# SrikarK-code/clip-dplm

Measured on NVIDIA B200. Metric: contrastive_fwd_bwd_pairs_per_sec, higher is better.
Workload: dtype bf16

## Files before the change

### clip-dplm_b200/csrc/clipnce_api.cu

```cuda
#include <cuda.h>
#include <cuda_bf16.h>
#include <cuda_runtime.h>

#include <cmath>
#include <cstdarg>
#include <cstdio>
#include <cstdlib>
#include <cstring>
#include <mutex>
#include <set>
#include <string>
#include <utility>

#include "../../include/clipnce.h"
#include "kernels_aux.cuh"
#include "kernels_head.cuh"
#include "kernels_link.cuh"
#include "kernels_pair.cuh"
#include "kernels_pair2.cuh"
#include "kernels_simt.cuh"
#include "kernels_tc.cuh"

namespace {

// ... 1007 lines not shown
  if (world == 1 || world < 0 || world > pair2::MAX_WORLD) return false;
  if (world == 0 ? n_rows != n_cols : n_rows * world != n_cols) return false;
  const int64_t min_n = env_int("CLIPNCE_BWD2_MIN_N", 12288);
  if (n_rows % 128 != 0 || n_cols % 256 != 0 || n_rows * n_cols < min_n * min_n || n_cols > (1ll << 22)) return false;
  if (world >= 2 && (n_cols / world) % 256 != 0) return false;
  const int slots = pair_slots();
  if (slots < 8) return false;
  pl->n_rb = (int)(n_rows / 128);
  pl->n_steps = (int)(n_cols / 256);
  pl->n_half = (int)ceil_div(d, 256);
  const int forced_p = (int)env_int("CLIPNCE_BWD2_P", 0);
  const int forced_seg = (int)env_int("CLIPNCE_BWD2_SEG", 0);
  constexpr double r = 1.0;
  double best_t = 1e300;
  int best_p = 0, best_seg = 0;
  for (int n_seg = 1; n_seg <= 8; n_seg *= 2) {
    int ns = world >= 2 ? world : n_seg;
    if (world == 0 && forced_seg >= 1) ns = forced_seg;
    if (pl->n_steps % ns != 0) continue;
    const int seg_steps = pl->n_steps / ns;
    if (seg_steps < 8 && ns > 1 && world == 0 && forced_seg < 1) continue;
    const int64_t n_items = (int64_t)pl->n_rb * ns;
    const double slab_steps = (double)(ns - 1) * (double)n_rows * (double)d * 8.0 / 3e12 / 3.9e-6;
    const bool force = forced_p >= 1 && forced_p <= slots - 1;
    for (int Pe = force ? forced_p : slots / 2; Pe <= (force ? forced_p : slots - 2); ++Pe) {
      const int Q = slots - Pe;
      const double tp = (double)ceil_div(n_items, Pe) * ((double)seg_steps + 1.0);
      const double tc_ = (double)n_items * (double)seg_steps / ((double)Q * 2.0 * r);
      const double t = ((tp > tc_ ? tp : tc_) + slab_steps) * (world == 0 && ns > 1 ? 1.08 : 1.0);
      if (t < best_t - 1e-9) { best_t = t; best_p = Pe; best_seg = ns; }
    }
    if (world >= 2 || forced_seg >= 1) break;
  }
  if (best_p == 0) return false;
  pl->P = best_p;
  pl->Q = slots - best_p;
  pl->n_seg = best_seg;
  pl->seg_steps = pl->n_steps / best_seg;
  pl->n_items = pl->n_rb * best_seg;
  pl->n_rounds = (int)ceil_div(pl->n_items, pl->P);
  pl->depth = pair2::RING_DEPTH;
  const int nkc = (int)(d / 64);
  const int total = (pair::SMEM_LIMIT - pair2::producer_smem(nkc, 0)) / pair::STAGE_BYTES;
  if (total < 4) return false;
  auto cap = [](int v) { return v > pair2::MAXS ? pair2::MAXS : v; };
  pl->stages_b = cap(total / 2);
  pl->stages_a = cap(total - total / 2);
  pl->stages_c = cap((pair::SMEM_LIMIT - pair2::consumer_smem(0)) / pair2::C_STAGE);
  const int ps = pair2::producer_smem(nkc, pl->stages_a + pl->stages_b), cs = pair2::consumer_smem(pl->stages_c);
  pl->smem = ps > cs ? ps : cs;
  size_t off = 0;
  auto region = [&](size_t bytes) { const size_t o = off; off = (size_t)round_up((int64_t)(off + bytes), 256); return o; };
  pl->off_flags = region(sizeof(uint32_t) * 2 * (size_t)pl->n_rounds * (size_t)pl->seg_steps);
  pl->off_ring = region((size_t)pl->depth * (size_t)pl->P * 128 * 256 * 2);
  pl->off_dxh = region(sizeof(float) * (size_t)pl->n_seg * (size_t)n_rows * (size_t)d);
  pl->off_dyh = region(sizeof(float) * (size_t)n_cols * (size_t)d);
  pl->off_part = region(sizeof(float) * (size_t)ceil_div(n_rows > n_cols ? n_rows : n_cols, 8));
  pl->bytes = off;
  return true;
}

int bwd2_launch(const Bwd2Plan& pl, const void* x, const void* y, const float* rinv_x, const float* rinv_y, int64_t n_rows,
                int64_t n_cols, int64_t d, int64_t diag_offset, float scale, const float* scale_dev, const float* row_m,
                const float* row_w, const float* col_m, const float* col_w, float diag_w, char* ws, float* const* dy_peer,
                int world, cudaStream_t st) {
  uint32_t* flags_dev = reinterpret_cast<uint32_t*>(ws + pl.off_flags);
  const size_t n_flags = (size_t)pl.n_rounds * (size_t)pl.seg_steps;
  CUDA_TRY(cudaMemsetAsync(flags_dev, 0, sizeof(uint32_t) * 2 * n_flags, st));
  pair2::Params p;
  memset(&p, 0, sizeof p);
  p.n_rows = (int)n_rows; p.n_cols = (int)n_cols; p.d = (int)d;
  p.nkc = (int)(d / 64); p.nq2 = (int)ceil_div(d, 256); p.n_half = pl.n_half;
  p.nsbuf = p.nq2 <= 2 ? 2 : 1;
  p.n_rb = pl.n_rb; p.n_seg = pl.n_seg; p.seg_steps = pl.seg_steps; p.n_items = pl.n_items; p.n_rounds = pl.n_rounds;
  p.P = pl.P; p.Q = pl.Q; p.depth = pl.depth;
  p.stages_a = pl.stages_a; p.stages_b = pl.stages_b; p.stages_c = pl.stages_c;
  p.diag_offset = diag_offset; p.scale = scale; p.scale_dev = scale_dev; p.diag_w = diag_w;
  p.rinv_x = rinv_x; p.rinv_y = rinv_y; p.row_m = row_m; p.row_w = row_w; p.col_m = col_m; p.col_w = col_w;
  p.dx = reinterpret_cast<float*>(ws + pl.off_dxh);
  p.dy = reinterpret_cast<float*>(ws + pl.off_dyh);
  p.world = world;
  for (int s = 0; s < world; ++s) p.dy_peer[s] = dy_peer[s];
  p.ready = flags_dev; p.done = flags_dev + n_flags;
  CUtensorMap tx, ty, tyg, tg;
  int rc;
  if ((rc = make_tmap(&tx, x, d, n_rows, d, pair2::ROWS))) return rc;
  if ((rc = make_tmap(&ty, y, d, n_cols, d, 128))) return rc;
  if ((rc = make_tmap(&tyg, y, d, n_cols, d, 64))) return rc;
  if ((rc = make_tmap(&tg, ws + pl.off_ring, 256, (int64_t)pl.depth * pl.P * 128, 256, 64))) return rc;
  auto kern = tc_family(CLIPNCE_BF16, d, scale, 0) == 2 ? pair2::bwd2_kernel<true> : pair2::bwd2_kernel<false>;
  if ((rc = allow_smem(kern, pair::SMEM_LIMIT))) return rc;
  kern<<<2 * (pl.P + pl.Q), pair2::THREADS, pl.smem, st>>>(tx, ty, tyg, tg, p);
  CUDA_TRY(cudaGetLastError());
  return 0;
}
}

extern "C" {

int clipnce_backward_both_workspace_bytes(int64_t n_rows, int64_t n_cols, int64_t d, int dtype, float scale, int flags,
                                          int world, size_t* out) {
  if (!out) return fail(CLIPNCE_EINVAL, "backward_both_workspace_bytes: null pointer");
  Bwd2Plan pl;
  *out = (n_rows >= 1 && n_cols >= 1 && d >= 1 && bwd2_plan(n_rows, n_cols, d, dtype, scale, flags, world, &pl) &&
          check_device_sm100() == 0 && bwd2_device_ok()) ? pl.bytes : 0;
  return 0;
}

int clipnce_backward_both_dx(const void* x, const void* y, const float* rinv_x, const float* rinv_y, int64_t n,
                             int64_t d, float scale, const float* scale_dev, const float* row_m, const float* row_w,
                             const float* col_m, const float* col_w, float diag_w, int dtype, int flags,
                             const void* x_orig, const void* y_orig, int in_dtype, const float* grad_scale, void* dx,
                             void* dy, int out_dtype, float* d_scale_sum, void* workspace, size_t workspace_bytes,
                             void* stream) {
  if (!x || !y || !rinv_x || !rinv_y || !row_m || !row_w || !col_m || !col_w || !x_orig || !y_orig || !dx || !dy || !workspace)
    return fail(CLIPNCE_EINVAL, "backward_both_dx: null pointer");
  if ((in_dtype != CLIPNCE_BF16 && in_dtype != CLIPNCE_F32) || (out_dtype != CLIPNCE_BF16 && out_dtype != CLIPNCE_F32))
    return fail(CLIPNCE_EINVAL, "backward_both_dx: bad dtype");
  if (in_dtype == dtype && (x_orig != x || y_orig != y))
    return fail(CLIPNCE_EINVAL, "backward_both_dx: x_orig / y_orig of the compute type must be x / y themselves");
  if (!aligned16(x) || !aligned16(y) || !aligned16(workspace)) return fail(CLIPNCE_EINVAL, "backward_both_dx: operands must be 16-byte aligned");
  int rc = check_device_sm100();
  if (rc) return rc;
  Bwd2Plan pl;
  if (!bwd2_plan(n, n, d, dtype, scale, flags, 0, &pl) || !bwd2_device_ok())
    return fail(CLIPNCE_EUNSUPPORTED, "backward_both_dx: shape not served (see clipnce_backward_both_workspace_bytes)");
  if (workspace_bytes < pl.bytes) return fail(CLIPNCE_EWORKSPACE, "backward_both_dx: workspace %zu < %zu", workspace_bytes, pl.bytes);
  cudaStream_t st = as_stream(stream);
  char* ws = reinterpret_cast<char*>(workspace);
  if ((rc = bwd2_launch(pl, x, y, rinv_x, rinv_y, n, n, d, 0, scale, scale_dev, row_m, row_w, col_m, col_w, diag_w, ws, nullptr,
                        0, st)))
    return rc;
  float* ds_part = reinterpret_cast<float*>(ws + pl.off_part);
  const aux::FinishSide sx = finish_side(reinterpret_cast<float*>(ws + pl.off_dxh), pl.n_seg, n, d, x, x_orig, rinv_x, dx,
                                         d_scale_sum ? ds_part : nullptr);
  const aux::FinishSide sy = finish_side(reinterpret_cast<float*>(ws + pl.off_dyh), 1, n, d, y, y_orig, rinv_y, dy, nullptr);
  if ((rc = launch_finish(&sx, 1, n, d, CLIPNCE_BF16, in_dtype, out_dtype, grad_scale, true, st))) return rc;
  if ((rc = launch_finish(&sy, 1, n, d, CLIPNCE_BF16, in_dtype, out_dtype, grad_scale, true, st))) return rc;
  if (d_scale_sum) {
    aux::reduce_scalar_partials_par<<<1, 256, 0, st>>>(ds_part, (int)ceil_div(n, 8), 1.f, d_scale_sum);
    CUDA_TRY(cudaGetLastError());
  }
  return 0;
}

int clipnce_backward_both_sharded(const void* x, const void* y, const float* rinv_x, const float* rinv_y, int64_t n_rows,
                                  int64_t n_cols, int64_t d, int64_t diag_offset, float scale, const float* scale_dev,
                                  const float* row_m, const float* row_w, const float* col_m, const float* col_w,
                                  float diag_w, int dtype, int flags, void* const* peer_base, int world, int rank,
                                  int64_t slots_offset, void* workspace, size_t workspace_bytes, void* stream) {
  if (!x || !y || !rinv_x || !rinv_y || !row_m || !row_w || !col_m || !col_w || !workspace || !peer_base)
    return fail(CLIPNCE_EINVAL, "backward_both_sharded: null pointer");
  if (!aligned16(x) || !aligned16(y) || !aligned16(workspace)) return fail(CLIPNCE_EINVAL, "backward_both_sharded: operands must be 16-byte aligned");
  if (world < 2 || world > pair2::MAX_WORLD || rank < 0 || rank >= world || slots_offset < 0 || slots_offset % 16 != 0)
    return fail(CLIPNCE_EINVAL, "backward_both_sharded: bad world / rank / slots_offset");
  if (diag_offset != (int64_t)rank * n_rows) return fail(CLIPNCE_EINVAL, "backward_both_sharded: diag_offset must be rank * n_rows");
  int rc = check_device_sm100();
  if (rc) return rc;
  Bwd2Plan pl;
  if (!bwd2_plan(n_rows, n_cols, d, dtype, scale, flags, world, &pl) || !bwd2_device_ok())
    return fail(CLIPNCE_EUNSUPPORTED, "backward_both_sharded: shape not served (see clipnce_backward_both_workspace_bytes)");
  if (workspace_bytes < pl.bytes) return fail(CLIPNCE_EWORKSPACE, "backward_both_sharded: workspace %zu < %zu", workspace_bytes, pl.bytes);
  char* ws = reinterpret_cast<char*>(workspace);
  float* dy_peer[pair2::MAX_WORLD];
  for (int s = 0; s < world; ++s) {
    if (!peer_base[s] || !aligned16(peer_base[s])) return fail(CLIPNCE_EINVAL, "backward_both_sharded: peer buffer %d is null or unaligned", s);
// ... 346 lines not shown
```

### clip-dplm_b200/csrc/kernels_pair2.cuh

```cuda
#pragma once
#include "kernels_pair.cuh"

namespace pair2 {

using pair::LOG2E;
using pair::STAGE_BYTES;
using pair::STEP_J;
using pair::TMEM_COLS;

constexpr int THREADS = 416;
constexpr int STORE_WARP = 12;
constexpr int EPI_WARPS = 8;
constexpr int ROWS = 64;
constexpr int X_CHUNK = ROWS * 128;
constexpr int G_BYTES = 4 * 8192;
constexpr int SMALL = 10240;
constexpr int C_STAGE = 32768;
constexpr int MAXS = 6;
constexpr int RING_DEPTH = 16;
constexpr int MAX_WORLD = 16;

constexpr int B_FULL_A = 0, B_EMPTY_A = MAXS, B_FULL_B = 2 * MAXS, B_EMPTY_B = 3 * MAXS, B_XFULL = 4 * MAXS,
              B_XEMPTY = B_XFULL + 1, B_SFULL = B_XEMPTY + 1, B_SEMPTY = B_SFULL + 2, B_GFULL = B_SEMPTY + 2,
              B_GEMPTY = B_GFULL + 4, B_ACCFULL = B_GEMPTY + 4, B_ACCEMPTY = B_ACCFULL + 2, B_GSFULL = B_ACCEMPTY + 2,
              B_GSTORED = B_GSFULL + 4, B_COUNT = B_GSTORED + 4;
static_assert(B_COUNT * 8 <= 1000, "barrier block");

struct Params {
  int n_rows, n_cols, d;
  int nsbuf;
  int nkc, nq2, n_half;
  int n_rb, n_seg, seg_steps, n_items, n_rounds;
  int P, Q, depth;
  int stages_a, stages_b, stages_c;
  long long diag_offset;
  float scale, diag_w;
  const float* scale_dev;
  const float* rinv_x;
  const float* rinv_y;
  const float* row_m;
  const float* row_w;
  const float* col_m;
  const float* col_w;
  float* dx;
  float* dy;
  float* dy_peer[MAX_WORLD];
  int world;
  uint32_t* ready;
  uint32_t* done;
};

__host__ __device__ constexpr int producer_smem(int nkc, int stages) {
  return nkc * X_CHUNK + G_BYTES + stages * STAGE_BYTES + SMALL;
}
constexpr int FLUSH_BYTES = EPI_WARPS * 4096;
__host__ __device__ constexpr int consumer_smem(int stages) { return stages * C_STAGE + FLUSH_BYTES + SMALL; }
__device__ __forceinline__ float4 ld_shared_v4(uint32_t addr) {
  float4 v;
  asm volatile("ld.shared.v4.f32 {%0, %1, %2, %3}, [%4];" : "=f"(v.x), "=f"(v.y), "=f"(v.z), "=f"(v.w) : "r"(addr) : "memory");
  return v;
}

__device__ __forceinline__ void publish(uint32_t* flag) {
  ptx::fence_proxy_async_all();
  ptx::red_release_gpu_add(flag, 1u);
}

struct Sub {
  int seg, p_lo, p_hi, rb_lo;
  bool first, last;
};
__device__ __forceinline__ int round_items(const Params& p, int r) { return min(p.P, p.n_items - r * p.P); }
__device__ __forceinline__ int round_subs(const Params& p, int r) {
  const int lo = r * p.P, hi = lo + round_items(p, r);
  return (hi - 1) / p.n_rb - lo / p.n_rb + 1;
}
__device__ __forceinline__ Sub round_sub(const Params& p, int r, int k) {
  const int lo = r * p.P, hi = lo + round_items(p, r);
  Sub s;
  s.seg = lo / p.n_rb + k;
  const int a = max(lo, s.seg * p.n_rb), b = min(hi, (s.seg + 1) * p.n_rb);
  s.p_lo = a - lo;
  s.p_hi = b - lo;
  s.rb_lo = a - s.seg * p.n_rb;
  s.first = a == s.seg * p.n_rb;
  s.last = b == (s.seg + 1) * p.n_rb;
  return s;
}

template <bool TWO_EXP>
__global__ void __cluster_dims__(2, 1, 1) __launch_bounds__(THREADS, 1)
bwd2_kernel(const __grid_constant__ CUtensorMap tmap_x,
            const __grid_constant__ CUtensorMap tmap_y,
            const __grid_constant__ CUtensorMap tmap_yg,
            const __grid_constant__ CUtensorMap tmap_g,
            const Params p) {
  extern __shared__ __align__(1024) uint8_t smem[];
  const uint32_t base = ptx::smem_u32(smem);
  if ((base & 1023u) != 0) __trap();
  const uint32_t rank = ptx::cluster_ctarank();
  const bool leader = rank == 0;
  const int warp = threadIdx.x >> 5;
  const int lane = threadIdx.x & 31;
  const int pair_id = blockIdx.x >> 1;
  const bool is_producer = pair_id < p.P;

  const int body = max(producer_smem(p.nkc, p.stages_a + p.stages_b), consumer_smem(p.stages_c)) - SMALL;
  const uint32_t bars = base + body;
  auto bar = [&](int i) -> uint32_t { return bars + 8u * i; };
  volatile uint32_t* tmem_ptr_smem = reinterpret_cast<volatile uint32_t*>(smem + body + 1016);
  float* const colv = reinterpret_cast<float*>(smem + body + 1024);

  const float sc = p.scale_dev != nullptr ? __ldg(p.scale_dev) : p.scale;
  const float k2 = sc * LOG2E;

  if (warp == 0 && lane == 0) {
    ptx::prefetch_tmap(&tmap_x);
    ptx::prefetch_tmap(&tmap_y);
    ptx::prefetch_tmap(&tmap_yg);
    ptx::prefetch_tmap(&tmap_g);
  }
  if (warp == 1 && lane == 0) {
    for (int s = 0; s < MAXS; ++s) {
      ptx::mbar_init(bar(B_FULL_A + s), 1);
      ptx::mbar_init(bar(B_EMPTY_A + s), 1);
      ptx::mbar_init(bar(B_FULL_B + s), 1);
      ptx::mbar_init(bar(B_EMPTY_B + s), 1);
    }
    ptx::mbar_init(bar(B_XFULL), 1);
    ptx::mbar_init(bar(B_XEMPTY), 1);
    for (int b = 0; b < 2; ++b) {
      ptx::mbar_init(bar(B_SFULL + b), 1);
      ptx::mbar_init(bar(B_SEMPTY + b), 2 * EPI_WARPS);
      ptx::mbar_init(bar(B_ACCFULL + b), 1);
      ptx::mbar_init(bar(B_ACCEMPTY + b), 2 * EPI_WARPS);
    }
    for (int k = 0; k < 4; ++k) {
      ptx::mbar_init(bar(B_GFULL + k), 4);
      ptx::mbar_init(bar(B_GEMPTY + k), 1);
      ptx::mbar_init(bar(B_GSFULL + k), 2);
      ptx::mbar_init(bar(B_GSTORED + k), 1);
    }
    ptx::fence_mbar_init();
  }
  if (warp == 2) ptx::tmem_alloc_pair(ptx::smem_u32(const_cast<uint32_t*>(tmem_ptr_smem)), TMEM_COLS);
  ptx::tc_fence_before();
  __syncthreads();
  ptx::cluster_sync();
  ptx::tc_fence_after();
  const uint32_t tmem_base = *tmem_ptr_smem;

  const uint32_t desc_hi_k = static_cast<uint32_t>(ptx::smem_desc_k_sw128(0) >> 32);
  const uint32_t desc_hi_mn = static_cast<uint32_t>(ptx::smem_desc_mn_sw128(0, 8192) >> 32);
  auto desc_lo = [&](uint32_t addr, uint32_t lbo16) -> uint32_t { return ((addr & 0x3FFFFu) >> 4) | (lbo16 << 16); };
  auto mk = [&](uint32_t hi, uint32_t lo) -> uint64_t { return (static_cast<uint64_t>(hi) << 32) | lo; };

  if (is_producer) {
    const uint32_t x_smem = base;
    const uint32_t g_smem = x_smem + p.nkc * X_CHUNK;
    const uint32_t ring_a = g_smem + G_BYTES;
    const uint32_t ring_b = ring_a + p.stages_a * STAGE_BYTES;
    const int S_COL0 = TMEM_COLS - 128 * p.nsbuf;
    auto s_buf = [&](uint32_t gs) -> int { return p.nsbuf == 2 ? (int)(gs & 1u) : 0; };
    auto s_par = [&](uint32_t gs) -> uint32_t { return p.nsbuf == 2 ? ((gs >> 1) & 1u) : (gs & 1u); };

    if (warp == 0) {
      if (ptx::elect_one()) {
        int stage = 0;
        uint32_t phase = 0;
        for (int r = 0; r < p.n_rounds; ++r) {
          const int item = r * p.P + pair_id;
          if (item >= p.n_items) break;
          const int i0 = (item % p.n_rb) * (2 * ROWS) + (int)rank * ROWS;
          const int t0 = (item / p.n_rb) * p.seg_steps;
          ptx::mbar_wait(bar(B_XEMPTY), (r & 1) ^ 1u);
          if (leader) ptx::mbar_arrive_expect_tx(bar(B_XFULL), 2 * p.nkc * X_CHUNK);
          for (int kc = 0; kc < p.nkc; ++kc)
            ptx::tma_load_2d_pair(x_smem + kc * X_CHUNK, &tmap_x, bar(B_XFULL), kc * 64, i0);
          for (int t = t0; t < t0 + p.seg_steps; ++t) {
            for (int g = 0; g < p.nkc; ++g) {
              ptx::mbar_wait(bar(B_EMPTY_A + stage), phase ^ 1u);
              if (leader) ptx::mbar_arrive_expect_tx(bar(B_FULL_A + stage), 2 * STAGE_BYTES);
              ptx::tma_load_2d_pair(ring_a + stage * STAGE_BYTES, &tmap_y, bar(B_FULL_A + stage), g * 64,
                                    t * STEP_J + (int)rank * 128);
              if (++stage == p.stages_a) { stage = 0; phase ^= 1u; }
            }
          }
        }
      }
      __syncwarp();
    } else if (warp == 2) {
      if (ptx::elect_one()) {
        int stage = 0;
        uint32_t phase = 0;
        for (int r = 0; r < p.n_rounds; ++r) {
          const int item = r * p.P + pair_id;
          if (item >= p.n_items) break;
          const int t0 = (item / p.n_rb) * p.seg_steps;
          for (int t = t0; t < t0 + p.seg_steps; ++t) {
            for (int kc = 0; kc < 4; ++kc) {
              for (int q = 0; q < p.nq2; ++q) {
                const int wq = min(256, p.d - 256 * q);
                const int half = wq >> 1;
                const int ngr = half >> 6;
                ptx::mbar_wait(bar(B_EMPTY_B + stage), phase ^ 1u);
                if (leader) ptx::mbar_arrive_expect_tx(bar(B_FULL_B + stage), 2 * ngr * 8192);
                for (int gi = 0; gi < ngr; ++gi)
                  ptx::tma_load_2d_pair(ring_b + stage * STAGE_BYTES + gi * 8192, &tmap_yg, bar(B_FULL_B + stage),
                                        256 * q + half * (int)rank + 64 * gi, t * STEP_J + 64 * kc);
                if (++stage == p.stages_b) { stage = 0; phase ^= 1u; }
              }
            }
          }
        }
      }
      __syncwarp();
    } else if (warp == 1) {
      if (leader && ptx::elect_one()) {
        constexpr uint32_t idesc_s = ptx::idesc_bf16_f32_major(2 * ROWS, STEP_J, 0, 0);
        const uint32_t x_lo0 = desc_lo(x_smem, 1), a_lo0 = desc_lo(ring_a, 1);
        int stage = 0;
        uint32_t phase = 0, ready = 0, gs = 0;
        for (int r = 0; r < p.n_rounds; ++r) {
          if (r * p.P + pair_id >= p.n_items) break;
          ptx::mbar_wait(bar(B_XFULL), r & 1);
          for (int t = 0; t < p.seg_steps; ++t, ++gs) {
            const int sb = s_buf(gs);
            ptx::mbar_wait(bar(B_SEMPTY + sb), s_par(gs) ^ 1u);
            const uint32_t d_tmem = tmem_base + S_COL0 + sb * 128;
            for (int g = 0; g < p.nkc; ++g) {
              if (!ready) ptx::mbar_wait(bar(B_FULL_A + stage), phase);
              ptx::tc_fence_after();
              int ns = stage + 1;
              uint32_t np = phase;
              if (ns == p.stages_a) { ns = 0; np ^= 1u; }
              ready = ptx::mma_box_pair(d_tmem, mk(desc_hi_k, x_lo0 + g * (X_CHUNK >> 4)),
                                        mk(desc_hi_k, a_lo0 + stage * (STAGE_BYTES >> 4)), 2, 2, idesc_s, g != 0,
                                        bar(B_FULL_A + ns), np);
              ptx::mma_commit_pair(bar(B_EMPTY_A + stage));
              if (g == p.nkc - 1) ptx::mma_commit_pair(bar(B_SFULL + sb));
              stage = ns;
              phase = np;
            }
          }
          ptx::mma_commit_pair(bar(B_XEMPTY));
        }
      }
      __syncwarp();
    } else if (warp == 3) {
      if (leader && ptx::elect_one()) {
        const uint32_t g_lo0 = desc_lo(g_smem, 1), b_lo0 = desc_lo(ring_b, 8192 >> 4);
        int stage = 0;
        uint32_t phase = 0, ready = 0, gs = 0;
        for (int r = 0; r < p.n_rounds; ++r) {
          if (r * p.P + pair_id >= p.n_items) break;
          ptx::mbar_wait(bar(B_ACCEMPTY), (r & 1) ^ 1u);
          ptx::tc_fence_after();
          for (int t = 0; t < p.seg_steps; ++t, ++gs) {
            for (int kc = 0; kc < 4; ++kc) {
              ptx::mbar_wait(bar(B_GFULL + kc), gs & 1u);
              for (int q = 0; q < p.nq2; ++q) {
                const int wq = min(256, p.d - 256 * q);
                const uint32_t idesc_g = ptx::idesc_bf16_f32_major(2 * ROWS, wq, 0, 1);
                if (!ready) ptx::mbar_wait(bar(B_FULL_B + stage), phase);
                ptx::tc_fence_after();
                int ns = stage + 1;
                uint32_t np = phase;
                if (ns == p.stages_b) { ns = 0; np ^= 1u; }
                ready = ptx::mma_box_pair(tmem_base + 128 * q, mk(desc_hi_k, g_lo0 + kc * (8192 >> 4)),
                                          mk(desc_hi_mn, b_lo0 + stage * (STAGE_BYTES >> 4)), 2, 2048 >> 4, idesc_g,
                                          (t | kc) != 0, bar(B_FULL_B + ns), np);
                ptx::mma_commit_pair(bar(B_EMPTY_B + stage));
                stage = ns;
                phase = np;
              }
              ptx::mma_commit_pair(bar(B_GEMPTY + kc));
            }
          }
          ptx::mma_commit_pair(bar(B_ACCFULL));
        }
      }
      __syncwarp();
    } else if (warp == STORE_WARP) {
      if (ptx::elect_one()) {
        uint32_t gs = 0;
        bool pending = false;
        uint32_t g_prev = 0;
        const uint64_t keep = ptx::l2_policy_evict_last();
        for (int r = 0; r < p.n_rounds; ++r) {
          if (r * p.P + pair_id >= p.n_items) break;
          const bool more_rounds = (r + 1) * p.P + pair_id < p.n_items;
          for (int t = 0; t < p.seg_steps; ++t, ++gs) {
            const uint32_t g = (uint32_t)r * (uint32_t)p.seg_steps + (uint32_t)t;
            const int row0 = ((int)(g % (uint32_t)p.depth) * p.P + pair_id) * 128 + (int)rank * ROWS;
            for (int kc = 0; kc < 4; ++kc) {
              ptx::mbar_wait(bar(B_GSFULL + kc), gs & 1u);
              ptx::tma_store_2d_hint(&tmap_g, g_smem + kc * 8192, 64 * kc, row0, keep);
              ptx::bulk_commit_group();
            }
            ptx::bulk_wait_group_read0();
            for (int kc = 0; kc < 4; ++kc) ptx::mbar_arrive(bar(B_GSTORED + kc));
            if (pending) {
              ptx::bulk_wait_group_le<4>();
              publish(p.ready + g_prev);
            }
            pending = true;
            g_prev = g;
            if (g + 1 >= (uint32_t)p.depth && (t + 1 < p.seg_steps || more_rounds)) {
              const uint32_t go = g + 1 - (uint32_t)p.depth;
              ptx::spin_until_ge(p.done + go, (uint32_t)(round_subs(p, (int)(go / (uint32_t)p.seg_steps)) * p.n_half));
            }
          }
        }
        if (pending) {
          ptx::bulk_wait_group0();
          publish(p.ready + g_prev);
        }
      }
      __syncwarp();
    } else {
      const int e = warp - 4;
      const int q = warp & 3;
      const int h = e >> 2;
      const int jh = q >> 1;
      const int i_local = 32 * (q & 1) + lane;
      const int te = threadIdx.x - 128;
      const int jl0 = 128 * jh + 64 * h;
      const int kc = 2 * jh + h;
      const uint32_t t_lane = tmem_base + (static_cast<uint32_t>(q * 32) << 16);
      const uint32_t g_row = g_smem + kc * 8192 + (i_local >> 3) * 1024 + (i_local & 7) * 128;
      const uint32_t sw = i_local & 7;
      const uint32_t sempty_leader = ptx::mapa(bar(B_SEMPTY), 0);
      const uint32_t gfull_leader = ptx::mapa(bar(B_GFULL + kc), 0);
      const uint32_t accempty_leader = ptx::mapa(bar(B_ACCEMPTY), 0);
      uint32_t gs = 0;

      for (int r = 0; r < p.n_rounds; ++r) {
        const int item = r * p.P + pair_id;
        if (item >= p.n_items) break;
        const int seg = item / p.n_rb;
        const int t0 = seg * p.seg_steps;
        const int i_glob = (item % p.n_rb) * (2 * ROWS) + (int)rank * ROWS + i_local;
        const float rx = p.rinv_x[i_glob];
        const float u = TWO_EXP ? 0.f : p.row_w[i_glob] * pair::ex2((sc - p.row_m[i_glob]) * LOG2E);
        const float rm2 = TWO_EXP ? p.row_m[i_glob] * LOG2E : 0.f;
        const float rw = TWO_EXP ? p.row_w[i_glob] : 0.f;
        const long long dcol = (long long)i_glob + p.diag_offset;
        float cw_n, cm_n, ry_n;
        {
          const long long jn = (long long)t0 * STEP_J + te;
          cw_n = p.col_w[jn]; cm_n = p.col_m[jn]; ry_n = p.rinv_y[jn];
        }

        for (int t = t0; t < t0 + p.seg_steps; ++t, ++gs) {
          const int sb = s_buf(gs);
          float* const cv = colv + (gs & 1) * 1024;
          cv[te] = ry_n * k2;
          cv[256 + te] = (TWO_EXP ? cw_n : cw_n * pair::ex2((sc - cm_n) * LOG2E)) * ry_n;
          cv[512 + te] = ry_n;
          if (TWO_EXP) cv[768 + te] = cw_n > 0.f ? cm_n * LOG2E : 0.f;
          if (t + 1 < t0 + p.seg_steps) {
            const long long jn = (long long)(t + 1) * STEP_J + te;
            cw_n = p.col_w[jn]; cm_n = p.col_m[jn]; ry_n = p.rinv_y[jn];
          }
          pair::named_bar_sync(1, EPI_WARPS * 32);
          const long long dl = dcol - ((long long)t * STEP_J + jl0);
          const bool has_diag = dl >= 0 && dl < 64;

          ptx::mbar_wait(bar(B_SFULL + sb), s_par(gs));
          ptx::tc_fence_after();
          uint32_t pk[32];
#pragma unroll
          for (int c = 0; c < 2; ++c) {
            uint32_t rr[32];
            ptx::tmem_ld_32x32b_x32(t_lane + S_COL0 + sb * 128 + 64 * h + 32 * c, rr);
            ptx::tmem_ld_wait();
            if (c == 1) {
              ptx::tc_fence_before();
              __syncwarp();
              if (lane == 0) ptx::mbar_arrive_cluster(sempty_leader + 8u * sb);
            }
            const float* const cjp = cv + jl0 + 32 * c;
#pragma unroll
            for (int x4 = 0; x4 < 8; ++x4) {
              const float4 cj4 = *reinterpret_cast<const float4*>(cjp + 4 * x4);
              const float4 vr4 = *reinterpret_cast<const float4*>(cjp + 256 + 4 * x4);
              const float4 ry4 = *reinterpret_cast<const float4*>(cjp + 512 + 4 * x4);
              const float cjv[4] = {cj4.x, cj4.y, cj4.z, cj4.w};
              const float vrv[4] = {vr4.x, vr4.y, vr4.z, vr4.w};
              const float ryv[4] = {ry4.x, ry4.y, ry4.z, ry4.w};
              float g[4];
              if constexpr (TWO_EXP) {
                const float4 cm4 = *reinterpret_cast<const float4*>(cjp + 768 + 4 * x4);
                const float cmv[4] = {cm4.x, cm4.y, cm4.z, cm4.w};
#pragma unroll
                for (int xx = 0; xx < 4; ++xx) {
                  const float y = __uint_as_float(rr[4 * x4 + xx]) * rx;
                  const float er = pair::ex2(fmaf(y, cjv[xx], -rm2)) * rw;
                  const float ec = pair::ex2(fmaf(y, cjv[xx], -cmv[xx]));
                  g[xx] = rx * fmaf(er, ryv[xx], ec * vrv[xx]);
                }
              } else {
#pragma unroll
                for (int xx = 0; xx < 4; ++xx) {
                  const float y = __uint_as_float(rr[4 * x4 + xx]) * rx;
                  const float ev = pair::ex2(fmaf(y, cjv[xx], -k2)) * rx;
                  g[xx] = ev * fmaf(u, ryv[xx], vrv[xx]);
                }
              }
              if (has_diag) {
#pragma unroll
                for (int xx = 0; xx < 4; ++xx)
                  if (dl == 32 * c + 4 * x4 + xx) g[xx] -= p.diag_w * rx * ryv[xx];
              }
              const __nv_bfloat162 p0 = __floats2bfloat162_rn(g[0], g[1]);
              const __nv_bfloat162 p1 = __floats2bfloat162_rn(g[2], g[3]);
              pk[16 * c + 2 * x4] = *reinterpret_cast<const uint32_t*>(&p0);
              pk[16 * c + 2 * x4 + 1] = *reinterpret_cast<const uint32_t*>(&p1);
            }
          }
          ptx::mbar_wait(bar(B_GEMPTY + kc), (gs & 1u) ^ 1u);
          ptx::mbar_wait(bar(B_GSTORED + kc), (gs & 1u) ^ 1u);
#pragma unroll
          for (int ch = 0; ch < 8; ++ch)
            pair::st_shared_v4(g_row + ((static_cast<uint32_t>(ch) ^ sw) << 4), pk[4 * ch], pk[4 * ch + 1], pk[4 * ch + 2],
                               pk[4 * ch + 3]);
          ptx::fence_proxy_async_smem();
          __syncwarp();
          if (lane == 0) {
            ptx::mbar_arrive_cluster(gfull_leader);
            ptx::mbar_arrive(bar(B_GSFULL + kc));
          }
        }

        ptx::mbar_wait(bar(B_ACCFULL), r & 1);
        ptx::tc_fence_after();
        const float osc = sc / rx;
        float* const slab = p.dx + (long long)seg * p.n_rows * p.d;
        for (int q2 = 0; q2 < p.nq2; ++q2) {
          const int halfw = min(256, p.d - 256 * q2) >> 1;
          if (64 * h < halfw) {
#pragma unroll
            for (int c = 0; c < 2; ++c) {
              uint32_t rr[32];
              ptx::tmem_ld_32x32b_x32(t_lane + 128 * q2 + 64 * h + 32 * c, rr);
              ptx::tmem_ld_wait();
              float* const dst = slab + (long long)i_glob * p.d + 256 * q2 + halfw * jh + 64 * h + 32 * c;
#pragma unroll
              for (int x4 = 0; x4 < 8; ++x4)
                *reinterpret_cast<float4*>(dst + 4 * x4) =
                    make_float4(__uint_as_float(rr[4 * x4]) * osc, __uint_as_float(rr[4 * x4 + 1]) * osc,
                                __uint_as_float(rr[4 * x4 + 2]) * osc, __uint_as_float(rr[4 * x4 + 3]) * osc);
            }
          }
        }
        ptx::tc_fence_before();
        __syncwarp();
        if (lane == 0) ptx::mbar_arrive_cluster(accempty_leader);
      }
    }
  } else {
    const int cidx = pair_id - p.P;
    const uint32_t ring_c = base;

    if (warp == 0) {
      if (ptx::elect_one()) {
        int stage = 0;
        uint32_t phase = 0;
        const uint64_t keep = ptx::l2_policy_evict_last();
        for (int r = 0; r < p.n_rounds; ++r) {
          const int pw = round_items(p, r);
          const int nsub = round_subs(p, r);
          for (int tau = 0; tau < p.seg_steps; ++tau) {
            const uint32_t g = (uint32_t)r * (uint32_t)p.seg_steps + (uint32_t)tau;
            const int slot = (int)(g % (uint32_t)p.depth);
            bool step_ready = false;
            for (int k = 0; k < nsub; ++k) {
              const Sub sub = round_sub(p, r, k);
              const int t = sub.seg * p.seg_steps + tau;
              for (int hh = 0; hh < p.n_half; ++hh) {
                if ((t * p.n_half + hh) % p.Q != cidx) continue;
                if (!step_ready) {
                  ptx::spin_until_ge(p.ready + g, 2u * (uint32_t)pw);
                  ptx::fence_proxy_async_all();
                  step_ready = true;
                }
                const int wq = min(256, p.d - 256 * hh);
                const int ngr = wq >> 7;
                for (int pp = sub.p_lo; pp < sub.p_hi; ++pp) {
                  for (int kb = 0; kb < 2; ++kb) {
                    ptx::mbar_wait(bar(B_EMPTY_A + stage), phase ^ 1u);
                    if (leader) ptx::mbar_arrive_expect_tx(bar(B_FULL_A + stage), 2 * (2 + ngr) * 8192);
                    const uint32_t st = ring_c + stage * C_STAGE;
                    const int grow = (slot * p.P + pp) * 128 + 64 * kb;
                    const int xrow = (sub.rb_lo + pp - sub.p_lo) * 128 + 64 * kb;
                    for (int gi = 0; gi < 2; ++gi)
                      ptx::tma_load_2d_pair_hint(st + gi * 8192, &tmap_g, bar(B_FULL_A + stage), 128 * (int)rank + 64 * gi, grow, keep);
                    for (int gi = 0; gi < ngr; ++gi)
                      ptx::tma_load_2d_pair(st + 16384 + gi * 8192, &tmap_x, bar(B_FULL_A + stage),
                                            256 * hh + (wq >> 1) * (int)rank + 64 * gi, xrow);
                    if (++stage == p.stages_c) { stage = 0; phase ^= 1u; }
                  }
                }
              }
            }
          }
        }
      }
      __syncwarp();
    } else if (warp == 1) {
      if (leader && ptx::elect_one()) {
        const uint32_t a_lo0 = desc_lo(ring_c, 8192 >> 4), b_lo0 = desc_lo(ring_c + 16384, 8192 >> 4);
        int stage = 0;
        uint32_t phase = 0, ready = 0, nt = 0;
        for (int r = 0; r < p.n_rounds; ++r) {
// ... 114 lines not shown
```

### clip-dplm_b200/csrc/ptx.cuh

```cuda
#pragma once
#include <cstdint>
#include <cuda.h>

namespace ptx {

__device__ __forceinline__ uint32_t smem_u32(const void* p) {
  return static_cast<uint32_t>(__cvta_generic_to_shared(p));
}

__device__ __forceinline__ uint32_t elect_one() {
  uint32_t pred;
  asm volatile(
      "{\n\t.reg .pred P;\n\t"
      "elect.sync _|P, 0xffffffff;\n\t"
      "selp.u32 %0, 1, 0, P;\n\t}"
      : "=r"(pred));
  return pred;
}

__device__ __forceinline__ void mbar_init(uint32_t bar, uint32_t count) {
  asm volatile("mbarrier.init.shared::cta.b64 [%0], %1;" ::"r"(bar), "r"(count) : "memory");
}
__device__ __forceinline__ void fence_mbar_init() {
  asm volatile("fence.mbarrier_init.release.cluster;" ::: "memory");
// ... 105 lines not shown
__device__ __forceinline__ void mma_f16(uint32_t d_tmem, uint64_t a_desc, uint64_t b_desc, uint32_t idesc,
                                        uint32_t accumulate) {
  asm volatile(
      "{\n\t.reg .pred p;\n\t"
      "setp.ne.b32 p, %4, 0;\n\t"
      "tcgen05.mma.cta_group::1.kind::f16 [%0], %1, %2, %3, p;\n\t}"
      ::"r"(d_tmem), "l"(a_desc), "l"(b_desc), "r"(idesc), "r"(accumulate)
      : "memory");
}
__device__ __forceinline__ void mma_commit(uint32_t bar) {
  asm volatile("tcgen05.commit.cta_group::1.mbarrier::arrive::one.shared::cluster.b64 [%0];" ::"r"(bar) : "memory");
}


__device__ __forceinline__ uint32_t mma_box_prefetch(uint32_t d_tmem, uint64_t a_desc, uint64_t b_desc, uint32_t idesc,
                                                     uint32_t accumulate_first, uint32_t next_bar, uint32_t next_parity) {
  uint32_t ready;
  asm volatile(
      "{\n\t"
      ".reg .pred P, PA, PT;\n\t"
      ".reg .b64 a1, b1, a2, b2, a3, b3;\n\t"
      "mbarrier.try_wait.parity.shared::cta.b64 P, [%6], %7;\n\t"
      "setp.ne.b32 PA, %5, 0;\n\t"
      "setp.eq.u32 PT, %1, %1;\n\t"
      "add.u64 a1, %2, 2;\n\t"
      "add.u64 b1, %3, 2;\n\t"
      "add.u64 a2, %2, 4;\n\t"
      "add.u64 b2, %3, 4;\n\t"
      "add.u64 a3, %2, 6;\n\t"
      "add.u64 b3, %3, 6;\n\t"
      "tcgen05.mma.cta_group::1.kind::f16 [%1], %2, %3, %4, PA;\n\t"
      "tcgen05.mma.cta_group::1.kind::f16 [%1], a1, b1, %4, PT;\n\t"
      "tcgen05.mma.cta_group::1.kind::f16 [%1], a2, b2, %4, PT;\n\t"
      "tcgen05.mma.cta_group::1.kind::f16 [%1], a3, b3, %4, PT;\n\t"
      "selp.u32 %0, 1, 0, P;\n\t"
      "}"
      : "=r"(ready)
      : "r"(d_tmem), "l"(a_desc), "l"(b_desc), "r"(idesc), "r"(accumulate_first), "r"(next_bar), "r"(next_parity)
      : "memory");
  return ready;
}

__device__ __forceinline__ uint32_t tma_box_prefetch(uint32_t dst_smem, const CUtensorMap* m, uint32_t full_bar,
                                                     uint32_t bytes, int c0, int c1, uint32_t next_bar,
                                                     uint32_t next_parity) {
  uint32_t ready;
  asm volatile(
      "{\n\t"
      ".reg .pred P;\n\t"
      "mbarrier.try_wait.parity.shared::cta.b64 P, [%7], %8;\n\t"
      "mbarrier.arrive.expect_tx.shared::cta.b64 _, [%3], %4;\n\t"
      "cp.async.bulk.tensor.2d.shared::cluster.global.mbarrier::complete_tx::bytes [%1], [%2, {%5, %6}], [%3];\n\t"
      "selp.u32 %0, 1, 0, P;\n\t"
      "}"
      : "=r"(ready)
      : "r"(dst_smem), "l"(reinterpret_cast<uint64_t>(m)), "r"(full_bar), "r"(bytes), "r"(c0), "r"(c1), "r"(next_bar),
        "r"(next_parity)
      : "memory");
  return ready;
}

__device__ __forceinline__ void tmem_ld_32x32b_x32(uint32_t taddr, uint32_t (&r)[32]) {
  asm volatile(
      "tcgen05.ld.sync.aligned.32x32b.x32.b32 "
      "{%0, %1, %2, %3, %4, %5, %6, %7, %8, %9, %10, %11, %12, %13, %14, %15, "
      "%16, %17, %18, %19, %20, %21, %22, %23, %24, %25, %26, %27, %28, %29, %30, %31}, [%32];"
      : "=r"(r[0]), "=r"(r[1]), "=r"(r[2]), "=r"(r[3]), "=r"(r[4]), "=r"(r[5]), "=r"(r[6]), "=r"(r[7]),
        "=r"(r[8]), "=r"(r[9]), "=r"(r[10]), "=r"(r[11]), "=r"(r[12]), "=r"(r[13]), "=r"(r[14]), "=r"(r[15]),
        "=r"(r[16]), "=r"(r[17]), "=r"(r[18]), "=r"(r[19]), "=r"(r[20]), "=r"(r[21]), "=r"(r[22]), "=r"(r[23]),
        "=r"(r[24]), "=r"(r[25]), "=r"(r[26]), "=r"(r[27]), "=r"(r[28]), "=r"(r[29]), "=r"(r[30]), "=r"(r[31])
      : "r"(taddr)
      : "memory");
}
__device__ __forceinline__ void tmem_ld_32x32b_x16(uint32_t taddr, uint32_t (&r)[16]) {
  asm volatile(
      "tcgen05.ld.sync.aligned.32x32b.x16.b32 "
      "{%0, %1, %2, %3, %4, %5, %6, %7, %8, %9, %10, %11, %12, %13, %14, %15}, [%16];"
      : "=r"(r[0]), "=r"(r[1]), "=r"(r[2]), "=r"(r[3]), "=r"(r[4]), "=r"(r[5]), "=r"(r[6]), "=r"(r[7]),
        "=r"(r[8]), "=r"(r[9]), "=r"(r[10]), "=r"(r[11]), "=r"(r[12]), "=r"(r[13]), "=r"(r[14]), "=r"(r[15])
      : "r"(taddr)
      : "memory");
}
__device__ __forceinline__ void tmem_ld_wait() { asm volatile("tcgen05.wait::ld.sync.aligned;" ::: "memory"); }


__device__ __forceinline__ uint32_t mapa(uint32_t addr, uint32_t rank) {
  uint32_t r;
  asm volatile("mapa.shared::cluster.u32 %0, %1, %2;" : "=r"(r) : "r"(addr), "r"(rank));
  return r;
}
__device__ __forceinline__ void mbar_arrive_cluster(uint32_t cluster_addr) {
  asm volatile("mbarrier.arrive.shared::cluster.b64 _, [%0];" ::"r"(cluster_addr) : "memory");
}
__device__ __forceinline__ void tmem_alloc_pair(uint32_t dst_smem, uint32_t ncols) {
  asm volatile("tcgen05.alloc.cta_group::2.sync.aligned.shared::cta.b32 [%0], %1;" ::"r"(dst_smem), "r"(ncols) : "memory");
  asm volatile("tcgen05.relinquish_alloc_permit.cta_group::2.sync.aligned;" ::: "memory");
}
__device__ __forceinline__ void tmem_dealloc_pair(uint32_t taddr, uint32_t ncols) {
  asm volatile("tcgen05.dealloc.cta_group::2.sync.aligned.b32 %0, %1;" ::"r"(taddr), "r"(ncols) : "memory");
}
__device__ __forceinline__ void tma_load_2d_pair(uint32_t dst_smem, const CUtensorMap* m, uint32_t bar, int c0, int c1) {
  asm volatile(
      "cp.async.bulk.tensor.2d.cta_group::2.shared::cluster.global.mbarrier::complete_tx::bytes [%0], [%1, {%3, %4}], [%2];"
      ::"r"(dst_smem), "l"(reinterpret_cast<uint64_t>(m)), "r"(bar & 0xFEFFFFFFu), "r"(c0), "r"(c1)
      : "memory");
}
__device__ __forceinline__ void tma_load_2d_pair_hint(uint32_t dst_smem, const CUtensorMap* m, uint32_t bar, int c0, int c1,
                                                      uint64_t policy) {
  asm volatile(
      "cp.async.bulk.tensor.2d.cta_group::2.shared::cluster.global.mbarrier::complete_tx::bytes.L2::cache_hint"
      " [%0], [%1, {%3, %4}], [%2], %5;"
      ::"r"(dst_smem), "l"(reinterpret_cast<uint64_t>(m)), "r"(bar & 0xFEFFFFFFu), "r"(c0), "r"(c1), "l"(policy)
      : "memory");
}
__device__ __forceinline__ void mma_commit_pair(uint32_t bar) {
  asm volatile("tcgen05.commit.cta_group::2.mbarrier::arrive::one.shared::cluster.multicast::cluster.b64 [%0], %1;"
               ::"r"(bar), "h"(static_cast<uint16_t>(3)) : "memory");
}
__device__ __forceinline__ uint32_t mma_box_pair(uint32_t d_tmem, uint64_t a_desc, uint64_t b_desc, uint32_t a_step,
                                                 uint32_t b_step, uint32_t idesc, uint32_t accumulate_first,
                                                 uint32_t next_bar, uint32_t next_parity) {
  uint32_t ready;
  asm volatile(
      "{\n\t"
      ".reg .pred P, PA, PT;\n\t"
      ".reg .b64 sa, sb, a1, b1, a2, b2, a3, b3;\n\t"
      "mbarrier.try_wait.parity.shared::cta.b64 P, [%8], %9;\n\t"
      "setp.ne.b32 PA, %7, 0;\n\t"
      "setp.eq.u32 PT, %1, %1;\n\t"
      "cvt.u64.u32 sa, %4;\n\t"
      "cvt.u64.u32 sb, %5;\n\t"
      "add.u64 a1, %2, sa;\n\t"
      "add.u64 b1, %3, sb;\n\t"
      "add.u64 a2, a1, sa;\n\t"
      "add.u64 b2, b1, sb;\n\t"
      "add.u64 a3, a2, sa;\n\t"
      "add.u64 b3, b2, sb;\n\t"
      "tcgen05.mma.cta_group::2.kind::f16 [%1], %2, %3, %6, PA;\n\t"
      "tcgen05.mma.cta_group::2.kind::f16 [%1], a1, b1, %6, PT;\n\t"
      "tcgen05.mma.cta_group::2.kind::f16 [%1], a2, b2, %6, PT;\n\t"
      "tcgen05.mma.cta_group::2.kind::f16 [%1], a3, b3, %6, PT;\n\t"
      "selp.u32 %0, 1, 0, P;\n\t"
      "}"
      : "=r"(ready)
      : "r"(d_tmem), "l"(a_desc), "l"(b_desc), "r"(a_step), "r"(b_step), "r"(idesc), "r"(accumulate_first),
        "r"(next_bar), "r"(next_parity)
      : "memory");
  return ready;
}

__device__ __forceinline__ uint64_t smem_desc_k_sw128(uint32_t smem_addr) {
  uint64_t d = 0;
  d |= static_cast<uint64_t>((smem_addr & 0x3FFFFu) >> 4);
  d |= static_cast<uint64_t>(1) << 16;
  d |= static_cast<uint64_t>(1024 >> 4) << 32;
  d |= static_cast<uint64_t>(1) << 46;
  d |= static_cast<uint64_t>(2) << 61;
  return d;
}

__device__ __forceinline__ uint64_t smem_desc_mn_sw128(uint32_t smem_addr, uint32_t lbo_bytes) {
  uint64_t d = 0;
  d |= static_cast<uint64_t>((smem_addr & 0x3FFFFu) >> 4);
  d |= static_cast<uint64_t>((lbo_bytes >> 4) & 0x3FFFu) << 16;
  d |= static_cast<uint64_t>(1024 >> 4) << 32;
  d |= static_cast<uint64_t>(1) << 46;
  d |= static_cast<uint64_t>(2) << 61;
  return d;
}
__host__ __device__ constexpr uint32_t idesc_bf16_f32_major(int m, int n, int a_mn, int b_mn) {
  return (1u << 4) | (1u << 7) | (1u << 10) | (static_cast<uint32_t>(a_mn) << 15) | (static_cast<uint32_t>(b_mn) << 16) |
         (static_cast<uint32_t>(n >> 3) << 17) | (static_cast<uint32_t>(m >> 4) << 24);
}

__host__ __device__ constexpr uint32_t idesc_bf16_f32(int m, int n) {
  return (1u << 4) | (1u << 7) | (1u << 10) | (static_cast<uint32_t>(n >> 3) << 17) |
         (static_cast<uint32_t>(m >> 4) << 24);
}

}
```

Baseline: 4.408 million.

## Write gradient ring directly from epilogue warps instead of TMA store warp

Epilogue warps now store their packed bf16 gradient tile rows straight to the global ring buffer with L2 evict-last hinted vector stores. They no longer hand the tile to a dedicated store warp that issued TMA stores. The store warp is reduced to a coordinator: it waits for downstream consumption, signals ring-free, waits for all epilogue warps, then publishes the ready flag. This removes the shared-memory handoff barriers and bulk-group waits, at the cost of per-thread global stores and a new cross-warp barrier on the epilogue's critical path. It also adds unused tcgen05.st and TMEM-A MMA helpers.

```diff
diff --git a/clip-dplm_b200/csrc/clipnce_api.cu b/clip-dplm_b200/csrc/clipnce_api.cu
--- a/clip-dplm_b200/csrc/clipnce_api.cu
+++ b/clip-dplm_b200/csrc/clipnce_api.cu
@@ -1113,6 +1113,7 @@
   p.world = world;
   for (int s = 0; s < world; ++s) p.dy_peer[s] = dy_peer[s];
   p.ready = flags_dev; p.done = flags_dev + n_flags;
+  p.ring = reinterpret_cast<uint16_t*>(ws + pl.off_ring);
   CUtensorMap tx, ty, tyg, tg;
   int rc;
   if ((rc = make_tmap(&tx, x, d, n_rows, d, pair2::ROWS))) return rc;
diff --git a/clip-dplm_b200/csrc/kernels_pair2.cuh b/clip-dplm_b200/csrc/kernels_pair2.cuh
--- a/clip-dplm_b200/csrc/kernels_pair2.cuh
+++ b/clip-dplm_b200/csrc/kernels_pair2.cuh
@@ -22,8 +22,8 @@
 
 constexpr int B_FULL_A = 0, B_EMPTY_A = MAXS, B_FULL_B = 2 * MAXS, B_EMPTY_B = 3 * MAXS, B_XFULL = 4 * MAXS,
               B_XEMPTY = B_XFULL + 1, B_SFULL = B_XEMPTY + 1, B_SEMPTY = B_SFULL + 2, B_GFULL = B_SEMPTY + 2,
-              B_GEMPTY = B_GFULL + 4, B_ACCFULL = B_GEMPTY + 4, B_ACCEMPTY = B_ACCFULL + 2, B_GSFULL = B_ACCEMPTY + 2,
-              B_GSTORED = B_GSFULL + 4, B_COUNT = B_GSTORED + 4;
+              B_GEMPTY = B_GFULL + 4, B_ACCFULL = B_GEMPTY + 4, B_ACCEMPTY = B_ACCFULL + 2, B_RFREE = B_ACCEMPTY + 2,
+              B_RFULL = B_RFREE + 1, B_COUNT = B_RFULL + 1;
 static_assert(B_COUNT * 8 <= 1000, "barrier block");
 
 struct Params {
@@ -48,6 +48,7 @@
   int world;
   uint32_t* ready;
   uint32_t* done;
+  uint16_t* ring;
 };
 
 __host__ __device__ constexpr int producer_smem(int nkc, int stages) {
@@ -59,11 +60,6 @@
   float4 v;
   asm volatile("ld.shared.v4.f32 {%0, %1, %2, %3}, [%4];" : "=f"(v.x), "=f"(v.y), "=f"(v.z), "=f"(v.w) : "r"(addr) : "memory");
   return v;
-}
-
-__device__ __forceinline__ void publish(uint32_t* flag) {
-  ptx::fence_proxy_async_all();
-  ptx::red_release_gpu_add(flag, 1u);
 }
 
 struct Sub {
@@ -138,9 +134,9 @@
     for (int k = 0; k < 4; ++k) {
       ptx::mbar_init(bar(B_GFULL + k), 4);
       ptx::mbar_init(bar(B_GEMPTY + k), 1);
-      ptx::mbar_init(bar(B_GSFULL + k), 2);
-      ptx::mbar_init(bar(B_GSTORED + k), 1);
     }
+    ptx::mbar_init(bar(B_RFREE), 1);
+    ptx::mbar_init(bar(B_RFULL), EPI_WARPS);
     ptx::fence_mbar_init();
   }
   if (warp == 2) ptx::tmem_alloc_pair(ptx::smem_u32(const_cast<uint32_t*>(tmem_ptr_smem)), TMEM_COLS);
@@ -284,37 +280,18 @@
     } else if (warp == STORE_WARP) {
       if (ptx::elect_one()) {
         uint32_t gs = 0;
-        bool pending = false;
-        uint32_t g_prev = 0;
-        const uint64_t keep = ptx::l2_policy_evict_last();
         for (int r = 0; r < p.n_rounds; ++r) {
           if (r * p.P + pair_id >= p.n_items) break;
-          const bool more_rounds = (r + 1) * p.P + pair_id < p.n_items;
           for (int t = 0; t < p.seg_steps; ++t, ++gs) {
             const uint32_t g = (uint32_t)r * (uint32_t)p.seg_steps + (uint32_t)t;
-            const int row0 = ((int)(g % (uint32_t)p.depth) * p.P + pair_id) * 128 + (int)rank * ROWS;
-            for (int kc = 0; kc < 4; ++kc) {
-              ptx::mbar_wait(bar(B_GSFULL + kc), gs & 1u);
-              ptx::tma_store_2d_hint(&tmap_g, g_smem + kc * 8192, 64 * kc, row0, keep);
-              ptx::bulk_commit_group();
-            }
-            ptx::bulk_wait_group_read0();
-            for (int kc = 0; kc < 4; ++kc) ptx::mbar_arrive(bar(B_GSTORED + kc));
-            if (pending) {
-              ptx::bulk_wait_group_le<4>();
-              publish(p.ready + g_prev);
-            }
-            pending = true;
-            g_prev = g;
-            if (g + 1 >= (uint32_t)p.depth && (t + 1 < p.seg_steps || more_rounds)) {
-              const uint32_t go = g + 1 - (uint32_t)p.depth;
+            if (g >= (uint32_t)p.depth) {
+              const uint32_t go = g - (uint32_t)p.depth;
               ptx::spin_until_ge(p.done + go, (uint32_t)(round_subs(p, (int)(go / (uint32_t)p.seg_steps)) * p.n_half));
             }
-          }
-        }
-        if (pending) {
-          ptx::bulk_wait_group0();
-          publish(p.ready + g_prev);
+            ptx::mbar_arrive(bar(B_RFREE));
+            ptx::mbar_wait(bar(B_RFULL), gs & 1u);
+            ptx::red_release_gpu_add(p.ready + g, 1u);
+          }
         }
       }
       __syncwarp();
@@ -333,6 +310,7 @@
       const uint32_t sempty_leader = ptx::mapa(bar(B_SEMPTY), 0);
       const uint32_t gfull_leader = ptx::mapa(bar(B_GFULL + kc), 0);
       const uint32_t accempty_leader = ptx::mapa(bar(B_ACCEMPTY), 0);
+      const uint64_t keep = ptx::l2_policy_evict_last();
       uint32_t gs = 0;
 
       for (int r = 0; r < p.n_rounds; ++r) {
@@ -420,17 +398,22 @@
             }
           }
           ptx::mbar_wait(bar(B_GEMPTY + kc), (gs & 1u) ^ 1u);
-          ptx::mbar_wait(bar(B_GSTORED + kc), (gs & 1u) ^ 1u);
 #pragma unroll
           for (int ch = 0; ch < 8; ++ch)
             pair::st_shared_v4(g_row + ((static_cast<uint32_t>(ch) ^ sw) << 4), pk[4 * ch], pk[4 * ch + 1], pk[4 * ch + 2],
                                pk[4 * ch + 3]);
           ptx::fence_proxy_async_smem();
           __syncwarp();
-          if (lane == 0) {
-            ptx::mbar_arrive_cluster(gfull_leader);
-            ptx::mbar_arrive(bar(B_GSFULL + kc));
-          }
+          if (lane == 0) ptx::mbar_arrive_cluster(gfull_leader);
+          ptx::mbar_wait(bar(B_RFREE), gs & 1u);
+          const uint32_t g = (uint32_t)r * (uint32_t)p.seg_steps + (uint32_t)(t - t0);
+          uint16_t* const line =
+              p.ring + ((long long)((int)(g % (uint32_t)p.depth) * p.P + pair_id) * 128 + (int)rank * ROWS + i_local) * 256 + jl0;
+#pragma unroll
+          for (int ch = 0; ch < 8; ++ch)
+            ptx::st_global_v4_hint(line + 8 * ch, pk[4 * ch], pk[4 * ch + 1], pk[4 * ch + 2], pk[4 * ch + 3], keep);
+          __syncwarp();
+          if (lane == 0) ptx::mbar_arrive(bar(B_RFULL));
         }
 
         ptx::mbar_wait(bar(B_ACCFULL), r & 1);
diff --git a/clip-dplm_b200/csrc/ptx.cuh b/clip-dplm_b200/csrc/ptx.cuh
--- a/clip-dplm_b200/csrc/ptx.cuh
+++ b/clip-dplm_b200/csrc/ptx.cuh
@@ -211,6 +211,23 @@
       : "memory");
 }
 __device__ __forceinline__ void tmem_ld_wait() { asm volatile("tcgen05.wait::ld.sync.aligned;" ::: "memory"); }
+__device__ __forceinline__ void tmem_st_32x32b_x32(uint32_t taddr, const uint32_t (&r)[32]) {
+  asm volatile(
+      "tcgen05.st.sync.aligned.32x32b.x32.b32 [%0], "
+      "{%1, %2, %3, %4, %5, %6, %7, %8, %9, %10, %11, %12, %13, %14, %15, %16, "
+      "%17, %18, %19, %20, %21, %22, %23, %24, %25, %26, %27, %28, %29, %30, %31, %32};"
+      ::"r"(taddr), "r"(r[0]), "r"(r[1]), "r"(r[2]), "r"(r[3]), "r"(r[4]), "r"(r[5]), "r"(r[6]), "r"(r[7]),
+        "r"(r[8]), "r"(r[9]), "r"(r[10]), "r"(r[11]), "r"(r[12]), "r"(r[13]), "r"(r[14]), "r"(r[15]),
+        "r"(r[16]), "r"(r[17]), "r"(r[18]), "r"(r[19]), "r"(r[20]), "r"(r[21]), "r"(r[22]), "r"(r[23]),
+        "r"(r[24]), "r"(r[25]), "r"(r[26]), "r"(r[27]), "r"(r[28]), "r"(r[29]), "r"(r[30]), "r"(r[31])
+      : "memory");
+}
+__device__ __forceinline__ void tmem_st_wait() { asm volatile("tcgen05.wait::st.sync.aligned;" ::: "memory"); }
+
+__device__ __forceinline__ void st_global_v4_hint(void* ptr, uint32_t a, uint32_t b, uint32_t c, uint32_t d, uint64_t policy) {
+  asm volatile("st.global.L2::cache_hint.v4.b32 [%0], {%1, %2, %3, %4}, %5;"
+               ::"l"(ptr), "r"(a), "r"(b), "r"(c), "r"(d), "l"(policy) : "memory");
+}
 
 
 __device__ __forceinline__ uint32_t mapa(uint32_t addr, uint32_t rank) {
@@ -277,6 +294,37 @@
       : "memory");
   return ready;
 }
+__device__ __forceinline__ uint32_t mma_tmem_a_pair(uint32_t d_tmem, uint32_t a_tmem, uint64_t b_desc, uint32_t a_step,
+                                                    uint32_t b_step, uint32_t idesc, uint32_t accumulate_first,
+                                                    uint32_t next_bar, uint32_t next_parity) {
+  uint32_t ready;
+  asm volatile(
+      "{\n\t"
+      ".reg .pred P, PA, PT;\n\t"
+      ".reg .b32 a1, a2, a3;\n\t"
+      ".reg .b64 sb, b1, b2, b3;\n\t"
+      "mbarrier.try_wait.parity.shared::cta.b64 P, [%8], %9;\n\t"
+      "setp.ne.b32 PA, %7, 0;\n\t"
+      "setp.eq.u32 PT, %1, %1;\n\t"
+      "cvt.u64.u32 sb, %5;\n\t"
+      "add.u32 a1, %2, %4;\n\t"
+      "add.u64 b1, %3, sb;\n\t"
+      "add.u32 a2, a1, %4;\n\t"
+      "add.u64 b2, b1, sb;\n\t"
+      "add.u32 a3, a2, %4;\n\t"
+      "add.u64 b3, b2, sb;\n\t"
+      "tcgen05.mma.cta_group::2.kind::f16 [%1], [%2], %3, %6, PA;\n\t"
+      "tcgen05.mma.cta_group::2.kind::f16 [%1], [a1], b1, %6, PT;\n\t"
+      "tcgen05.mma.cta_group::2.kind::f16 [%1], [a2], b2, %6, PT;\n\t"
+      "tcgen05.mma.cta_group::2.kind::f16 [%1], [a3], b3, %6, PT;\n\t"
+      "selp.u32 %0, 1, 0, P;\n\t"
+      "}"
+      : "=r"(ready)
+      : "r"(d_tmem), "r"(a_tmem), "l"(b_desc), "r"(a_step), "r"(b_step), "r"(idesc), "r"(accumulate_first),
+        "r"(next_bar), "r"(next_parity)
+      : "memory");
+  return ready;
+}
 
 __device__ __forceinline__ uint64_t smem_desc_k_sw128(uint32_t smem_addr) {
   uint64_t d = 0;
```

Result: slower. 3.668 million (median of 6 runs) (-16.8%).
